# jacarvalho/mpd-public

Hardware: AMD Instinct MI355X
Metric: denoising-steps/s (higher is better)
Workload: dtype f32; 1 GPU; cfg2: EnvDense2D-RobotPointMass shape, 100 trajectories (1 context(s)) x H=64 x D=4, T=100 (+5) reverse steps, unguided, U-Net dim_mults (1, 2, 4, 8), one plan = one bench step; parallelism=single, denoising_steps_per_plan=105

## Files before the change

### include/mpdx.h

```cpp
#ifndef MPDX_H
#define MPDX_H

#include <stddef.h>
#include <stdint.h>

#ifdef __cplusplus
extern "C" {
#endif

#define MPDX_E_INVALID   (-1)
#define MPDX_E_NOTFOUND  (-2)
#define MPDX_E_STATE     (-3)

#define MPDX_MAX_LEVELS 8

typedef struct mpdx_unet mpdx_unet;

typedef struct mpdx_unet_cfg {
    int32_t state_dim;
    int32_t n_support_points;
    int32_t unet_input_dim;
    int32_t n_levels;
    int32_t dim_mults[MPDX_MAX_LEVELS];
    int32_t time_emb_dim;
// ... 148 lines not shown
    float    step;
    int32_t  max_nodes, max_iters, max_connect_steps, n_edge_checks;
    uint64_t seed;
} mpdx_rrt_opts;
int mpdx_rrt_connect(const mpdx_guide_params* gp, const mpdx_rrt_opts* opts, const float* start, const float* goal, float* nodes,
                     int32_t* parent, int32_t* count, int32_t* link, int32_t* iters, int n, void* stream);

int mpdx_rrt_paths(const mpdx_guide_params* gp, const float* start, const float* goal, const float* nodes, const int32_t* parent, const int32_t* link,
                   float* trajs_out, int32_t* path_len, int n, int max_nodes, int H, float dt, int n_edge_checks, int rounds, void* stream);

int mpdx_plan(mpdx_unet* u, const float* packed_dev, const float* timetab_dev, int T, const mpdx_step_coefs* coefs,
              int n_without_noise, float* x, const float* noise, const float* hard_start, const float* hard_goal,
              float* chain, int B, float* ws, const mpdx_guide_params* guide, int n_guide_steps, int t_start_guide,
              uint32_t* guide_flags, int n_per_ctx, uint64_t rng_seed, uint64_t rng_offset, void* stream);

int mpdx_unet_profile(mpdx_unet* u, const float* packed_dev, const float* timetab_dev, int T, const float* x, int t,
                      int B, float* ws, void* stream, int cap, float* ms_out, double* flops_out,
                      const char** names_out, int* n_out);
int mpdx_layer_trace(mpdx_unet* u, const float* packed_dev, const float* timetab_dev, const float* x, int layer, int B, float* ws,
                     void* stream, long long* stamps32);
int mpdx_fused_trace(mpdx_unet* u, const float* packed_dev, const float* timetab_dev, const float* x, int seg, int B,
                     float* ws, void* stream, long long* stamps_out, int cap, int* n_out, int* nops_out);
int mpdx_unet_time_units(mpdx_unet* u, const float* packed_dev, const float* timetab_dev, int T, const float* x, int t, int B,
                         float* ws, void* stream, int unit_first, int unit_last, int reps, float* ms_avg);
int mpdx_unet_time_without(mpdx_unet* u, const float* packed_dev, const float* timetab_dev, int T, const float* x, int t, int B,
                           float* ws, void* stream, unsigned long long skip_mask, int reps, float* ms_avg);
int mpdx_unet_unit_layer(const mpdx_unet* u, int B, int i);
int mpdx_unet_fused_program(const mpdx_unet* u, int seg);
double mpdx_unet_unit_bytes(const mpdx_unet* u, int B, int i);
int mpdx_unet_unit_is_pair(const mpdx_unet* u, int B, int i);
// ... 9 lines not shown
```

### mpd_public_amd/_lib.py

```python
from __future__ import annotations

import ctypes as C
from pathlib import Path

import os as _os

_LIB_PATH = Path(_os.environ["MPDX_LIB"]) if _os.environ.get("MPDX_LIB") else Path(__file__).resolve().parent / "libmpdx.so"
_lib = None

MAX_LEVELS = 8


class UnetCfg(C.Structure):
    _fields_ = [("state_dim", C.c_int32), ("n_support_points", C.c_int32), ("unet_input_dim", C.c_int32),
                ("n_levels", C.c_int32), ("dim_mults", C.c_int32 * MAX_LEVELS), ("time_emb_dim", C.c_int32)]


class StepCoefs(C.Structure):
    _fields_ = [("sqrt_recip_alphas_cumprod", C.c_float), ("sqrt_recipm1_alphas_cumprod", C.c_float),
                ("posterior_mean_coef1", C.c_float), ("posterior_mean_coef2", C.c_float),
                ("noise_scale", C.c_float), ("noise_std_extra", C.c_float),
                ("predict_epsilon", C.c_int32), ("clip_denoised", C.c_int32), ("ddim_k1", C.c_float), ("ddim_k2", C.c_float),
                ("guide_scale", C.c_float)]

# ... 40 lines not shown
    "mpdx_unet_num_params": (_i, [_vp]),
    "mpdx_unet_param_info": (_i, [_vp, _i, C.POINTER(C.c_char_p), C.POINTER(C.c_int32 * 3), C.POINTER(C.c_int32)]),
    "mpdx_unet_packed_floats": (_sz, [_vp]),
    "mpdx_unet_timetab_floats": (_sz, [_vp, _i]),
    "mpdx_unet_workspace_floats": (_sz, [_vp, _i]),
    "mpdx_unet_pack_param": (_i, [_vp, C.c_char_p, _vp, _sz, _vp, _vp]),
    "mpdx_unet_build_timetab": (_i, [_vp, _vp, _vp, _i, _vp, _vp]),
    "mpdx_unet_forward": (_i, [_vp, _vp, _vp, _i, _vp, _i, _vp, _i, _vp, _vp]),
    "mpdx_ddpm_step": (_i, [_vp, _vp, _vp, _i, _vp, _vp, _vp, _vp, C.POINTER(StepCoefs), _i, _i, _vp, _vp, _i, _i, _vp, _vp]),
    "mpdx_add_noise": (_i, [_vp, _vp, _vp, _vp, _f, _f, _vp, _i, _i, _i, _vp]),
    "mpdx_hard_conds": (_i, [_vp, _vp, _i, C.POINTER(C.c_int32), C.POINTER(_vp), _i, _i, _i, _vp]),
    "mpdx_q_sample": (_i, [_vp, _vp, _vp, _vp, _vp, _vp, _vp, _vp, _i, _i, _i, _i, _vp]),
    "mpdx_weighted_loss": (_i, [_vp, _vp, _vp, _vp, _vp, _i, _vp, _i, _i, _i, _vp]),
    "mpdx_plan": (_i, [_vp, _vp, _vp, _i, C.POINTER(StepCoefs), _i, _vp, _vp, _vp, _vp, _vp, _i, _vp,
                        C.POINTER(GuideParams), _i, _i, _vp, _i, C.c_uint64, C.c_uint64, _vp]),
    "mpdx_guide_step": (_i, [C.POINTER(GuideParams), _vp, _vp, _vp, _vp, _vp, _vp, _i, _i, _i, _i, _vp]),
    "mpdx_guide_step_scaled": (_i, [C.POINTER(GuideParams), _vp, _vp, _vp, _vp, _vp, _vp, _i, _i, _i, _i, _f, _vp]),
    "mpdx_guide_time": (_i, [C.POINTER(GuideParams), _vp, _vp, _vp, _i, _i, _i, _i, _i, _vp, C.POINTER(C.c_float)]),
    "mpdx_traj_metrics": (_i, [C.POINTER(GuideParams), _vp, _vp, _i, _i, _i, _i, _vp]),
    "mpdx_traj_metrics_mask": (_i, [C.POINTER(GuideParams), _vp, _vp, _vp, _i, _i, _i, _i, _vp]),
    "mpdx_guide_trace": (_i, [C.POINTER(GuideParams), _vp, _vp, _i, _i, _i, _vp, C.POINTER(C.c_longlong)]),
    "mpdx_absmax": (_i, [_vp, _vp, _i, _i, _i, _i, _vp]),
    "mpdx_sdf_grid_bake": (_i, [C.POINTER(GuideParams), _i, _vp, _vp, C.POINTER(C.c_int * 3), C.POINTER(C.c_float * 3), _f, _vp]),
    "mpdx_unet_profile": (_i, [_vp, _vp, _vp, _i, _vp, _i, _i, _vp, _vp, _i, C.POINTER(C.c_float), C.POINTER(C.c_double),
                                C.POINTER(C.c_char_p), C.POINTER(C.c_int)]),
    "mpdx_layer_trace": (_i, [_vp, _vp, _vp, _vp, _i, _i, _vp, _vp, C.POINTER(C.c_longlong)]),
    "mpdx_fused_trace": (_i, [_vp, _vp, _vp, _vp, _i, _i, _vp, _vp, C.POINTER(C.c_longlong), _i, C.POINTER(C.c_int), C.POINTER(C.c_int)]),
    "mpdx_unet_time_units": (_i, [_vp, _vp, _vp, _i, _vp, _i, _i, _vp, _vp, _i, _i, _i, C.POINTER(C.c_float)]),
    "mpdx_unet_time_without": (_i, [_vp, _vp, _vp, _i, _vp, _i, _i, _vp, _vp, C.c_uint64, _i, C.POINTER(C.c_float)]),
    "mpdx_unet_unit_layer": (_i, [_vp, _i, _i]),
# ... 66 lines not shown
```

### mpd_public_amd/csrc/fused_level.hpp

```cpp
#pragma once
#include "conv_block.hpp"
#include "fused_geom.hpp"

namespace mpdx {

#define MPDX_FUSED_SHAPES(X)                                                                                   \
    X(0, CONV_S1, 5, 1, 0, 32, 64, 1) X(1, CONV_S1, 5, 2, 1, 32, 64, 1) X(2, CONV_S1, 5, 2, 0, 32, 64, 1) X(3, CONV_DOWN, 3, 2, 0, 32, 32, 0)     \
    X(4, CONV_S1, 5, 2, 0, 64, 32, 1) X(5, CONV_S1, 5, 4, 2, 64, 32, 1) X(6, CONV_S1, 5, 4, 0, 64, 32, 1) X(7, CONV_DOWN, 3, 4, 0, 64, 16, 0)     \
    X(8, CONV_S1, 5, 16, 0, 64, 16, 1) X(9, CONV_S1, 5, 4, 16, 64, 16, 1) X(10, CONV_S1, 5, 4, 0, 64, 16, 1) X(11, CONV_UPT, 4, 4, 0, 64, 32, 0)  \
    X(12, CONV_S1, 5, 8, 0, 32, 32, 1) X(13, CONV_S1, 5, 2, 8, 32, 32, 1) X(14, CONV_S1, 5, 2, 0, 32, 32, 1) X(15, CONV_UPT, 4, 2, 0, 32, 64, 0) \
    X(16, CONV_S1, 5, 4, 0, 128, 16, 1) X(17, CONV_S1, 5, 8, 4, 128, 16, 1) X(18, CONV_S1, 5, 8, 0, 128, 16, 1) X(19, CONV_DOWN, 3, 8, 0, 128, 8, 0)
constexpr int kFusedShapeFinal = 63;

inline int fused_shape_id(int mode, int ks, int nc16, int rnc16, int cout, int L_out, int gn) {
#define X(id, M, K, N, R, CO, LO, G) if (mode == M && ks == K && nc16 == N && rnc16 == R && cout == CO && L_out == LO && gn == G) return id;
    MPDX_FUSED_SHAPES(X)
#undef X
    return -1;
}

constexpr int kFusedWaves = 4;
constexpr int kFusedThreads = 64 * kFusedWaves;

template <int MODE_, int KS_, int NC16_, int NCR_, int COUT_, int LOUT_, int GN_>
// ... 461 lines not shown
#pragma unroll
    for (int k = 0; k < kFinalPre; ++k) {
        const int idx = tid + k * kFusedThreads;
        if (k * kFusedThreads >= n) continue;
        const int ic = idx < n ? idx : 0;
        const int p = ic / a.D, d = ic - p * a.D;
        const size_t o = (size_t)b * n + ic;
        fp.xv[k] = a.x_in[o];
        if (a.fmode == 1 && !a.rng.on && a.noise) fp.nz[k] = a.noise[o];
        if (a.hs && p == 0) fp.hc[k] = a.hs[(size_t)b * a.D + d];
        if (a.hg && p == H - 1) fp.hc[k] = a.hg[(size_t)b * a.D + d];
    }
}

template <int CF = 0>
__device__ __forceinline__ void fused_final_op(const FusedArgs& a, const FusedLay& lay, const FusedOp& op, const FinalPre& fp, float* smem, int tid, int lane, int b) {
    f32x4* const sm4 = (f32x4*)smem;
    constexpr int NT_ = kFusedThreads;
    float vmax = 0.f;
    const int H = lay.H, n = H * a.D;
    const int Cf = CF ? CF : lay.Cf;
    const int wrs = Cf + 4;
    const float* const fw = smem + lay.par_off + lay.fpar_off;
    float nzr[kFinalPre];
    const bool coop = a.fmode == 1 && a.rng.on && (((a.rng.elem0 + (unsigned long long)b * (unsigned)n) & 3ull) == 0ull) && (n & 3) == 0;
    if (coop) {
        const int qidx = (tid & ~63) + (lane >> 4) * NT_ + (lane & 15) * 4;
        float z[4] = {0.f, 0.f, 0.f, 0.f};
        if (qidx < n) philox_normal4(a.rng.seed, a.rng.offset + ((a.rng.elem0 + (unsigned long long)b * (unsigned)n + (unsigned)qidx) >> 2), z);
#pragma unroll
        for (int k = 0; k < kFinalPre; ++k) {
// ... 34 lines not shown
                if (a.hs && p == 0) r = fp.hc[k];
                if (a.hg && p == H - 1) r = fp.hc[k];
            } else {
                if (a.k.clip_denoised) x0 = fminf(fmaxf(x0, -1.0f), 1.0f);
                r = __fadd_rn(__fmul_rn(a.k.posterior_mean_coef1, x0), __fmul_rn(a.k.posterior_mean_coef2, xv));
                if (a.fmode == 1) {
                    if (a.rng.on) r = __fadd_rn(r, __fmul_rn(__fmul_rn(a.k.noise_scale, coop ? nzr[k] : philox_normal_at(a.rng.seed, a.rng.offset, a.rng.elem0 + o)), a.k.noise_std_extra));
                    else if (a.noise) r = __fadd_rn(r, __fmul_rn(__fmul_rn(a.k.noise_scale, fp.nz[k]), a.k.noise_std_extra));
                    if (a.hs && p == 0) r = fp.hc[k];
                    if (a.hg && p == H - 1) r = fp.hc[k];
                }
            }
        }
        a.out[o] = r;
        if (a.chain) a.chain[o] = r;
        vmax = fmaxf(vmax, fabsf(r));
    }
    if (a.absmax) {
#pragma unroll
        for (int s = 32; s >= 1; s >>= 1) vmax = fmaxf(vmax, __shfl_xor(vmax, s, 64));
        if (lane == 0) atomicMax(a.absmax + b / a.n_per_ctx, __float_as_uint(vmax));
    }
}

template <bool SAVE>
__global__ __launch_bounds__(kFusedThreads) void fused_level_kernel(const FusedArgs a) {
#ifndef MPDX_NO_WARM_KERNARG
    warm_kernarg<(int)sizeof(FusedArgs)>();
#endif
    extern __shared__ __attribute__((aligned(16))) float smem[];
// ... 71 lines not shown
        }
        fused_conv_op<typename FusedShapeOf<SH>::type, SAVE>(a, lay, op, ring, smem, wave, lane, b, nbase, nmax, tr_base, tr);
    }
}

template <class GEOM_, int... SH>
struct FusedSeq {
    using GEOM = GEOM_;
    static constexpr int N = sizeof...(SH);
    static constexpr int ids[sizeof...(SH)] = {SH...};
    template <int I>
    static constexpr int prev_cout() {
        if constexpr (I > 0 && ids[I > 0 ? I - 1 : 0] != kFusedShapeFinal) return FusedShapeOf<ids[I > 0 ? I - 1 : 0]>::type::COUT;
        else return 0;
    }
    template <int I, bool SAVE>
    __device__ static __forceinline__ void run_from(const FusedArgs& a, const FusedLay& lay, f32x4 (&ring)[kFusedRing], FinalPre& fp, float* smem, int tid, int wave,
                                                    int lane, int b, long long* tr_base, int& tr) {
        if constexpr (I < N) {
            fused_static_op<GEOM, ids[I], I, (I + 1 < N ? ids[I + 1 < N ? I + 1 : I] : -1), prev_cout<I>(), SAVE>(a, lay, ring, fp, smem, tid, wave, lane, b, tr_base, tr);
            run_from<I + 1, SAVE>(a, lay, ring, fp, smem, tid, wave, lane, b, tr_base, tr);
        }
    }
};

template <class SEQ, bool SAVE = false>
__global__ __launch_bounds__(kFusedThreads) void fused_program_kernel(const FusedArgs a) {
#ifndef MPDX_NO_WARM_KERNARG
    warm_kernarg<(int)sizeof(FusedArgs)>();
#endif
    extern __shared__ __attribute__((aligned(16))) float smem[];
    const int tid = threadIdx.x, lane = tid & 63;
    const int wave = __builtin_amdgcn_readfirstlane(tid >> 6);
    const int b = blockIdx.x;
    int tr = 0;
    long long* const tr_base = (MPDX_TRACE_PTR(a.trace) && b == 0 && lane == 0) ? a.trace + wave * 128 : nullptr;
// ... 2 lines not shown
    f32x4 ring[kFusedRing];
    FinalPre fp;
    const FusedLay lay = fused_lay<typename SEQ::GEOM>(a);
    fused_prologue<typename SEQ::GEOM>(a, lay, smem, ring, tid, lane, wave, b, tr_base, tr);
    SEQ::template run_from<0, SAVE>(a, lay, ring, fp, smem, tid, wave, lane, b, tr_base, tr);
}

using FusedSeqDown = FusedSeq<GeomDown, 0, 1, 2, 2, 3, 4, 5, 6, 6, 7>;
using FusedSeqUpA = FusedSeq<GeomNone, 8, 9, 10, 10, 11>;
using FusedSeqUpB = FusedSeq<GeomNone, 12, 13, 14, 14, 15, 2, kFusedShapeFinal>;
using FusedSeqUpAB = FusedSeq<GeomUpAB, 8, 9, 10, 10, 11, 12, 13, 14, 14, 15, 2, kFusedShapeFinal>;
using FusedSeqDown3 = FusedSeq<GeomDown3, 0, 1, 2, 2, 3, 4, 5, 6, 6, 7, 16, 17, 18, 18, 19>;
using FusedSeqMid2 = FusedSeq<GeomNone, 16, 17, 18, 18, 19>;
using FusedSeqMid3 = FusedSeq<GeomMid3, 16, 17, 18, 18, 18, 18, 18, 18>;

}
```

### mpd_public_amd/csrc/host.hpp

```cpp
#pragma once
#include <hip/hip_runtime.h>

#include <algorithm>
#include <cmath>
#include <cstdarg>
#include <cstdio>
#include <cstdlib>
#include <cstring>
#include <mutex>
#include <set>
#include <string>
#include <unordered_map>
#include <vector>

#include "../../include/mpdx.h"
#include "conv_block.hpp"
#include "conv_ws.hpp"
#include "fused_level.hpp"
#include "switches.hpp"
#include "train_types.hpp"

namespace mpdx {

int fail(int code, const char* fmt, ...);
// ... 109 lines not shown

int pick_row_stride(int cin_pad, int mode, int L_in, int L_out, int LP);
void choose_tile(const Layer& l, int B, int& MT, int& NT);
bool layer_ksplit(const Layer& l);
int check_ready(const mpdx_unet* u);
unsigned fused_mask(int B);
bool fused_save_variant(const mpdx_unet::Fused& f);
int ensure_fused_streams(mpdx_unet* u, const float* packed, hipStream_t st);
int claim_fused_stream_jobs(mpdx_unet* u, const float* packed, const void** jobs, int* n);
int launch_final_step(const FinalArgs& fa, hipStream_t st);
int launch_conv_layer(const Layer& l, ConvArgs& a, int B, hipStream_t st);
bool pair_tile(const Layer& l1, const Layer& l2, int B, int& MT, int& NT);
int launch_conv_pair(int MT, int NT, const ConvArgs& a1, const ConvArgs& a2, const Layer& l1, const Layer& l2, hipStream_t st);
int launch_weight_stationary(int variant, const Layer& l, ConvArgs& a, const ConvArgs& a2, int B, hipStream_t st);
int launch_fused_args(const mpdx_unet::Fused& f, const FusedArgs& a, int B, hipStream_t st, bool save = false);
int launch_fused_train(const mpdx_unet::Fused& f, const FusedArgs& a, int B, hipStream_t st);
struct NoiseRng;
int launch_guide(const mpdx_guide_params* gp, float* x, float* grad_out, const float* hs, const float* hg, const uint32_t* amax_in,
                 uint32_t* amax_out, int n_per_ctx, int B, int H, int D, hipStream_t st, const float* noise = nullptr, float noise_scale = 0.f,
                 float noise_extra = 0.f, float* chain = nullptr, float guide_scale = 1.0f, const NoiseRng* rng = nullptr);

}
```

### mpd_public_amd/csrc/k_fused.hip

```cpp
#include "host.hpp"

namespace mpdx {

int launch_fused_args(const mpdx_unet::Fused& f, const FusedArgs& a, int B, hipStream_t st, bool save) {
    if (save) return launch_fused_train(f, a, B, st);
    switch (f.program) {
        case 0:
            if (int rc = raise_lds_limit((const void*)fused_program_kernel<FusedSeqDown>)) return rc;
            hipLaunchKernelGGL(fused_program_kernel<FusedSeqDown>, dim3(B), dim3(kFusedThreads), f.lds_bytes, st, a);
            break;
        case 1:
            if (int rc = raise_lds_limit((const void*)fused_program_kernel<FusedSeqUpA>)) return rc;
            hipLaunchKernelGGL(fused_program_kernel<FusedSeqUpA>, dim3(B), dim3(kFusedThreads), f.lds_bytes, st, a);
            break;
        case 2:
            if (int rc = raise_lds_limit((const void*)fused_program_kernel<FusedSeqUpB>)) return rc;
            hipLaunchKernelGGL(fused_program_kernel<FusedSeqUpB>, dim3(B), dim3(kFusedThreads), f.lds_bytes, st, a);
            break;
        case 3:
            if (int rc = raise_lds_limit((const void*)fused_program_kernel<FusedSeqUpAB>)) return rc;
            hipLaunchKernelGGL(fused_program_kernel<FusedSeqUpAB>, dim3(B), dim3(kFusedThreads), f.lds_bytes, st, a);
            break;
        case 4:
            if (int rc = raise_lds_limit((const void*)fused_program_kernel<FusedSeqMid2>)) return rc;
// ... 2 lines not shown
        case 5:
            if (int rc = raise_lds_limit((const void*)fused_program_kernel<FusedSeqDown3>)) return rc;
            hipLaunchKernelGGL(fused_program_kernel<FusedSeqDown3>, dim3(B), dim3(kFusedThreads), f.lds_bytes, st, a);
            break;
        case 6:
            if (int rc = raise_lds_limit((const void*)fused_program_kernel<FusedSeqMid3>)) return rc;
            hipLaunchKernelGGL(fused_program_kernel<FusedSeqMid3>, dim3(B), dim3(kFusedThreads), f.lds_bytes, st, a);
            break;
        default:
            if (int rc = raise_lds_limit((const void*)fused_level_kernel<false>)) return rc;
            hipLaunchKernelGGL(fused_level_kernel<false>, dim3(B), dim3(kFusedThreads), f.lds_bytes, st, a);
    }
    return 0;
}

}
```

### mpd_public_amd/csrc/mpdx.hip

```cpp
#include "host.hpp"
#include "loss.hpp"

namespace mpdx {

static thread_local char g_err[512] = "";
int fail(int code, const char* fmt, ...) {
    va_list ap;
    va_start(ap, fmt);
    vsnprintf(g_err, sizeof(g_err), fmt, ap);
    va_end(ap);
    return code;
}

int raise_lds_limit(const void* kern) {
    static std::mutex mu;
    static std::set<std::pair<int, const void*>> done;
    int dev = 0;
    HIP_TRY(hipGetDevice(&dev));
    std::lock_guard<std::mutex> lock(mu);
    if (done.count({dev, kern})) return 0;
    HIP_TRY(hipFuncSetAttribute(kern, hipFuncAttributeMaxDynamicSharedMemorySize, 160 * 1024));
    done.insert({dev, kern});
    return 0;
}
// ... 991 lines not shown
        hipLaunchKernelGGL(restream_all_kernel, dim3(64, (unsigned)u->n_jobs), dim3(256), 0, st, const_cast<float*>(packed), (const CopyJobDev*)u->jobs_dev);
    HIP_TRY(hipGetLastError());
    u->streams_for = packed; u->streams_version = u->pack_version;
    return 0;
}
int claim_fused_stream_jobs(mpdx_unet* u, const float* packed, const void** jobs, int* n) {
    *jobs = nullptr; *n = 0;
    if (u->streams_for == packed && u->streams_version == u->pack_version) return 0;
    if (int rc = ensure_stream_jobs(u)) return rc;
    *jobs = u->jobs_dev; *n = u->n_jobs;
    u->streams_for = packed; u->streams_version = u->pack_version;
    return 0;
}

bool fused_save_variant(const mpdx_unet::Fused& f) { return f.program == 0 || f.program == 3 || f.program == 5 || f.program == 6 || f.program < 0; }
static int run_fused(mpdx_unet* u, const mpdx_unet::Fused& f, const float* packed, const float* tt_row, const float* x, float* ws,
                     int B, const FinalArgs* fa, hipStream_t st) {
    const size_t slot = u->slot_floats * (size_t)B;
    auto src = [&](int s) -> const float* { return s == SRC_X ? x : (s == SRC_NONE ? nullptr : ws + slot * s); };
    if (int rc = ensure_fused_streams(u, packed, st)) return rc;
    FusedArgs a = f.tmpl;
    a.packed = packed; a.tt_row = tt_row;
    a.gsrc1 = src(f.in1); a.gsrc2 = src(f.in2);
    a.gsrc3 = f.in3 != SRC_NONE ? src(f.in3) : a.gsrc1;
    for (int k = 0; k < 3; ++k) a.gout[k] = f.gout_slot[k] >= 0 ? ws + slot * f.gout_slot[k] : nullptr;
    a.B = B;
    a.trace = (g_fused_trace && (g_fused_trace_seg < 0 || g_fused_trace_seg == (int)(&f - &u->fused[0]))) ? g_fused_trace : nullptr;
    if (f.has_final) {
        if (!fa) return fail(MPDX_E_STATE, "fused final segment needs the step arguments");
        a.x_in = fa->x_in; a.noise = fa->noise; a.hs = fa->hs; a.hg = fa->hg; a.out = fa->out; a.chain = fa->chain;
        a.absmax = fa->absmax; a.fmode = fa->mode; a.n_per_ctx = fa->n_per_ctx > 0 ? fa->n_per_ctx : B; a.k = fa->k;
        a.rng = fa->rng;
    }
    return launch_fused_args(f, a, B, st);
}


static int run_unit(mpdx_unet* u, const mpdx_unet::Unit& un, const float* packed, const float* row, const float* x, float* ws, int B,
                    const FinalArgs* fa, hipStream_t st) {
    if (un.fused >= 0) return run_fused(u, u->fused[un.fused], packed, row, x, ws, B, fa, st);
    if (un.pair) return run_pair(u, u->layers[un.layer], u->layers[un.layer + 1], packed, row, x, ws, B, st);
    return run_layer(u, u->layers[un.layer], packed, row, x, ws, B, st);
}
static double unit_flops(const mpdx_unet* u, const mpdx_unet::Unit& un, int B) {
    if (un.fused >= 0) {
        const auto& f = u->fused[un.fused];
        double fl = 0.0;
        for (int k = f.first; k < f.first + f.count; ++k) fl += layer_flops(u->layers[k], B);
// ... 248 lines not shown
static int plan_side(mpdx_unet* u, mpdx_unet::PlanSide** out) {
    mpdx_unet::PlanSide& s = u->side;
    if (!s.stream) {
        HIP_TRY(hipStreamCreateWithFlags(&s.stream, hipStreamNonBlocking));
        HIP_TRY(hipEventCreateWithFlags(&s.fork, hipEventDisableTiming));
        HIP_TRY(hipEventCreateWithFlags(&s.join, hipEventDisableTiming));
    }
    *out = &s;
    return 0;
}
static int plan_split_point(int B, int npc, int n_ctx) {
    if (sw::plan_chains() != 2 || B < 16) return 0;
    if (n_ctx >= 2) return (n_ctx / 2) * npc;
    return std::min(B - 4, ((B / 2) + 3) & ~3);
}
}

int mpdx_plan(mpdx_unet* u, const float* packed, const float* timetab, int T, const mpdx_step_coefs* coefs, int n_without_noise,
              float* x, const float* noise, const float* hard_start, const float* hard_goal, float* chain, int B, float* ws,
              const mpdx_guide_params* guide, int n_guide_steps, int t_start_guide, uint32_t* guide_flags, int n_per_ctx,
              uint64_t rng_seed, uint64_t rng_offset, void* stream) {
    if (!u || !packed || !timetab || !coefs || !x || !ws || T <= 0 || n_without_noise < 0 || B <= 0)
        return fail(MPDX_E_INVALID, "bad argument");
    if (int rc = check_ready(u)) return rc;
    hipStream_t st = (hipStream_t)stream;
    const int H = u->cfg.n_support_points, D = u->cfg.state_dim;
    const size_t n = (size_t)B * H * D;
    const int npc = n_per_ctx > 0 ? n_per_ctx : B;
    const int n_ctx = (B + npc - 1) / npc;
    const int steps = T + n_without_noise;
// ... 10 lines not shown
    const int B0 = plan_split_point(B, npc, n_ctx);
    const int nch = B0 > 0 ? 2 : 1;
    mpdx_unet::PlanSide* side = nullptr;
    if (nch == 2) {
        if (int rc = plan_side(u, &side)) return rc;
        if (int rc = ensure_fused_streams(u, packed, st)) return rc;
        HIP_TRY(hipEventRecord(side->fork, st));
        HIP_TRY(hipStreamWaitEvent(side->stream, side->fork, 0));
    }
    const int b0[2] = {0, B0}, nb[2] = {nch == 2 ? B0 : B, B - B0};
    hipStream_t sts[2] = {st, side ? side->stream : st};
    float* wss[2] = {ws, ws + u->slot_floats * (size_t)nb[0] * u->n_slots};
    struct ChainsGuard { int* p; ~ChainsGuard() { *p = 1; } } guard{&g_plan_chains};
    g_plan_chains = nch;
    bool forked = nch == 2;
    int k = 0;
    for (int i = T - 1; i >= -n_without_noise; --i, ++k) {
        const int t = i < 0 ? 0 : i;
        const bool guided = guide && i < t_start_guide;
        const float* nz = (t == 0 || !noise) ? nullptr : noise + (size_t)k * n;
        NoiseRng rng;
        memset(&rng, 0, sizeof(rng));
        if (!noise && t != 0) { rng.on = 1; rng.seed = rng_seed; rng.offset = rng_offset; rng.elem0 = (unsigned long long)(k + 1) * n; }
        float* ch = chain ? chain + (size_t)(k + 1) * n : nullptr;
        uint32_t* fl = guided ? guide_flags + (size_t)k * (n_guide_steps + 1) * n_ctx : nullptr;
        if (nch == 2 && !forked) {
            HIP_TRY(hipEventRecord(side->fork, st));
            HIP_TRY(hipStreamWaitEvent(side->stream, side->fork, 0));
            forked = true;
        }
// ... 1 lines not shown
            const size_t eo = (size_t)b0[c] * H * D;
            FinalArgs fa;
            memset(&fa, 0, sizeof(fa));
            fa.x_in = x + eo; fa.out = x + eo;
            fa.k = coefs[t];
            fa.n_per_ctx = npc;
            if (!guided) {
                fa.rng = rng;
                fa.rng.elem0 += eo;
                fa.noise = nz ? nz + eo : nullptr;
                fa.hs = hard_start ? hard_start + (size_t)b0[c] * D : nullptr; fa.hg = hard_goal ? hard_goal + (size_t)b0[c] * D : nullptr;
                fa.chain = ch ? ch + eo : nullptr; fa.mode = 1;
            } else {
                fa.mode = 2; fa.absmax = fl + b0[c] / npc;
            }
            if (int rc = run_unet_and_final(u, packed, timetab, T, x + eo, t, nb[c], wss[c], fa, sts[c])) return rc;
        }
        if (guided) {
            if (nch == 2) {
                HIP_TRY(hipEventRecord(side->join, side->stream));
                HIP_TRY(hipStreamWaitEvent(st, side->join, 0));
                forked = false;
            }
            for (int j = 0; j < n_guide_steps; ++j) {
                const bool last = j == n_guide_steps - 1;
                if (int rc = launch_guide(guide, x, nullptr, hard_start, hard_goal, fl + (size_t)j * n_ctx, fl + (size_t)(j + 1) * n_ctx, npc, B, H,
                                          D, st, last ? nz : nullptr, coefs[t].noise_scale, coefs[t].noise_std_extra, last ? ch : nullptr,
                                          coefs[t].guide_scale, last ? &rng : nullptr))
                    return rc;
            }
// ... 2 lines not shown
            if (dbg >= 2) {
                hipError_t e = hipStreamSynchronize(st);
                if (e == hipSuccess && nch == 2) e = hipStreamSynchronize(side->stream);
                if (e != hipSuccess) return fail((int)e, "mpdx_plan: loop iteration %d (t=%d%s) faulted: %s", k, t, guided ? ", guided" : "", hipGetErrorString(e));
            }
            hipError_t e = hipGetLastError();
            if (e != hipSuccess) return fail((int)e, "mpdx_plan: launch in loop iteration %d (t=%d%s) failed: %s", k, t, guided ? ", guided" : "", hipGetErrorString(e));
        }
    }
    if (nch == 2 && forked) {
        HIP_TRY(hipEventRecord(side->join, side->stream));
        HIP_TRY(hipStreamWaitEvent(st, side->join, 0));
    }
    HIP_TRY(hipGetLastError());
    return 0;
}

int mpdx_unet_profile(mpdx_unet* u, const float* packed, const float* timetab, int T, const float* x, int t, int B, float* ws,
                      void* stream, int cap, float* ms_out, double* flops_out, const char** names_out, int* n_out) {
    if (!u || !packed || !timetab || !x || !ws || !ms_out || !n_out) return fail(MPDX_E_INVALID, "null argument");
    if (int rc = check_ready(u)) return rc;
    if (t < 0 || t >= T) return fail(MPDX_E_INVALID, "timestep %d outside [0,%d)", t, T);
    hipStream_t st = (hipStream_t)stream;
    bool fin_fused = false;
    const auto units = current_units(u, B, &fin_fused);
    const bool need_final = !fin_fused;
    const int nl = (int)units.size() + (need_final ? 1 : 0);
    if (cap < nl) return fail(MPDX_E_INVALID, "need room for %d launches", nl);
    static float* scratch = nullptr;
    static size_t scratch_n = 0;
// ... 275 lines not shown
```

### mpd_public_amd/diffusion_model.py

```python
from __future__ import annotations

from copy import copy

import torch
import torch.nn as nn

from . import _lib
from .sample_functions import apply_hard_conditioning, ddpm_sample_fn, extract, step_coefs
from .schedules import diffusion_buffers


def make_timesteps(batch_size, i, device):
    t = torch.full((batch_size,), i, device=device, dtype=torch.long)
    t._mpdx_value = int(i)
    t._mpdx_version = t._version
    return t


def timestep_hint(t):
    v = getattr(t, "_mpdx_value", None)
    return v if v is not None and getattr(t, "_mpdx_version", -1) == t._version else None


class GaussianDiffusionModel(nn.Module):
# ... 115 lines not shown
        npc = int(n_per_context or B)
        gp_ref, flags, n_gs, t_sg = None, None, 0, 0
        if int(n_guide_steps) <= 0:
            guide = None
        if guide is not None:
            import ctypes as C
            gp_ref = C.byref(guide.device_params(dev))
            n_gs = int(n_guide_steps)
            t_sg = int(min(t_start_guide, T + 1)) if t_start_guide != float("inf") else T + 1
            flags = torch.empty(steps * (n_gs + 1) * ((B + npc - 1) // npc), dtype=torch.int32, device=dev)
        _lib.check(_lib.load().mpdx_plan(hdl, packed.data_ptr(), tab.data_ptr(), T, coefs, n0,
                                         x.data_ptr(), noise_ptr, _lib.ptr(hs), _lib.ptr(hg), _lib.ptr(chain), B,
                                         ws.data_ptr(), gp_ref, n_gs, t_sg, _lib.ptr(flags), npc, rng_seed, rng_offset,
                                         _lib.current_stream()), "mpdx_plan")
        return x, chain

    def predict_noise_from_start(self, x_t, t, x0):
        if self.predict_epsilon:
            return x0
        return (extract(self.sqrt_recip_alphas_cumprod, t, x_t.shape) * x_t - x0) / extract(self.sqrt_recipm1_alphas_cumprod, t, x_t.shape)

    def predict_start_from_noise(self, x_t, t, noise):
        if not self.predict_epsilon:
            return noise
        return extract(self.sqrt_recip_alphas_cumprod, t, x_t.shape) * x_t - extract(self.sqrt_recipm1_alphas_cumprod, t, x_t.shape) * noise

    def q_posterior(self, x_start, x_t, t):
        mean = extract(self.posterior_mean_coef1, t, x_t.shape) * x_start + extract(self.posterior_mean_coef2, t, x_t.shape) * x_t
        return mean, extract(self.posterior_variance, t, x_t.shape), extract(self.posterior_log_variance_clipped, t, x_t.shape)

# ... 230 lines not shown
```

Measured before the change: 5733 denoising-steps/s.

## Merge up-path fused program with next step's down-path into one launch

Adds a fused_step_kernel that runs the final up-path fused program (including the DDPM update) and then, in the same block, the next timestep's down-path fused program. The updated sample goes straight into LDS as the next network input. This saves one kernel launch per denoising step and the global round trip of the sample between steps. A slot-redirection planner moves intermediate buffers when the down half would overwrite tensors the up half still reads. The merge only applies for a single chain, unguided runs and B no larger than the CU count. It raises LDS use per block and adds complex slot-aliasing logic.

```diff
diff --git a/include/mpdx.h b/include/mpdx.h
--- a/include/mpdx.h
+++ b/include/mpdx.h
@@ -186,6 +186,8 @@
               float* chain, int B, float* ws, const mpdx_guide_params* guide, int n_guide_steps, int t_start_guide,
               uint32_t* guide_flags, int n_per_ctx, uint64_t rng_seed, uint64_t rng_offset, void* stream);
 
+int mpdx_plan_merged_steps(mpdx_unet* u, int B, int T, int n_without_noise, int guided, int t_start_guide);
+
 int mpdx_unet_profile(mpdx_unet* u, const float* packed_dev, const float* timetab_dev, int T, const float* x, int t,
                       int B, float* ws, void* stream, int cap, float* ms_out, double* flops_out,
                       const char** names_out, int* n_out);
diff --git a/mpd_public_amd/_lib.py b/mpd_public_amd/_lib.py
--- a/mpd_public_amd/_lib.py
+++ b/mpd_public_amd/_lib.py
@@ -78,6 +78,7 @@
     "mpdx_weighted_loss": (_i, [_vp, _vp, _vp, _vp, _vp, _i, _vp, _i, _i, _i, _vp]),
     "mpdx_plan": (_i, [_vp, _vp, _vp, _i, C.POINTER(StepCoefs), _i, _vp, _vp, _vp, _vp, _vp, _i, _vp,
                         C.POINTER(GuideParams), _i, _i, _vp, _i, C.c_uint64, C.c_uint64, _vp]),
+    "mpdx_plan_merged_steps": (_i, [_vp, _i, _i, _i, _i, _i]),
     "mpdx_guide_step": (_i, [C.POINTER(GuideParams), _vp, _vp, _vp, _vp, _vp, _vp, _i, _i, _i, _i, _vp]),
     "mpdx_guide_step_scaled": (_i, [C.POINTER(GuideParams), _vp, _vp, _vp, _vp, _vp, _vp, _i, _i, _i, _i, _f, _vp]),
     "mpdx_guide_time": (_i, [C.POINTER(GuideParams), _vp, _vp, _vp, _i, _i, _i, _i, _i, _vp, C.POINTER(C.c_float)]),
diff --git a/mpd_public_amd/csrc/fused_level.hpp b/mpd_public_amd/csrc/fused_level.hpp
--- a/mpd_public_amd/csrc/fused_level.hpp
+++ b/mpd_public_amd/csrc/fused_level.hpp
@@ -499,7 +499,8 @@
 }
 
 template <int CF = 0>
-__device__ __forceinline__ void fused_final_op(const FusedArgs& a, const FusedLay& lay, const FusedOp& op, const FinalPre& fp, float* smem, int tid, int lane, int b) {
+__device__ __forceinline__ void fused_final_op(const FusedArgs& a, const FusedLay& lay, const FusedOp& op, const FinalPre& fp, float* smem, int tid, int lane, int b,
+                                               float* hand = nullptr, int hand_rs = 0) {
     f32x4* const sm4 = (f32x4*)smem;
     constexpr int NT_ = kFusedThreads;
     float vmax = 0.f;
@@ -564,6 +565,7 @@
         }
         a.out[o] = r;
         if (a.chain) a.chain[o] = r;
+        if (hand) hand[(p + 2) * hand_rs + d] = r;
         vmax = fmaxf(vmax, fabsf(r));
     }
     if (a.absmax) {
@@ -665,12 +667,12 @@
         if constexpr (I > 0 && ids[I > 0 ? I - 1 : 0] != kFusedShapeFinal) return FusedShapeOf<ids[I > 0 ? I - 1 : 0]>::type::COUT;
         else return 0;
     }
-    template <int I, bool SAVE>
+    template <int I, bool SAVE, int END = N>
     __device__ static __forceinline__ void run_from(const FusedArgs& a, const FusedLay& lay, f32x4 (&ring)[kFusedRing], FinalPre& fp, float* smem, int tid, int wave,
                                                     int lane, int b, long long* tr_base, int& tr) {
-        if constexpr (I < N) {
+        if constexpr (I < END) {
             fused_static_op<GEOM, ids[I], I, (I + 1 < N ? ids[I + 1 < N ? I + 1 : I] : -1), prev_cout<I>(), SAVE>(a, lay, ring, fp, smem, tid, wave, lane, b, tr_base, tr);
-            run_from<I + 1, SAVE>(a, lay, ring, fp, smem, tid, wave, lane, b, tr_base, tr);
+            run_from<I + 1, SAVE, END>(a, lay, ring, fp, smem, tid, wave, lane, b, tr_base, tr);
         }
     }
 };
@@ -703,4 +705,110 @@
 using FusedSeqMid2 = FusedSeq<GeomNone, 16, 17, 18, 18, 19>;
 using FusedSeqMid3 = FusedSeq<GeomMid3, 16, 17, 18, 18, 18, 18, 18, 18>;
 
-}
+constexpr int kStepUpBase = GeomDown3::g.par_off + GeomDown3::g.par_floats;
+constexpr int kStepUpFloats = 16000;
+
+struct FusedStepArgs {
+    const float* packed;
+    const float* tt_up;
+    const float* tt_dn;
+    const float* gsrc1; const float* gsrc2; const float* gsrc3;
+    float* gout[3];
+    const float* x_in; const float* noise; const float* hs; const float* hg;
+    float* out; float* chain;
+    int up_sbase[kMaxFusedOps], dn_sbase[kMaxFusedOps];
+    int up_gpar_off, up_par_floats, up_tt_lo, up_in_clear;
+    int dn_gpar_off, dn_tt_lo;
+    int D, B;
+    mpdx_step_coefs k;
+    NoiseRng rng;
+};
+
+static_assert(sizeof(FusedStepArgs) == 360, "DESIGN.md section 3 states this size");
+template <class UP, class DN>
+__global__ __launch_bounds__(kFusedThreads) __attribute__((amdgpu_waves_per_eu(3))) void fused_step_kernel(const FusedStepArgs m) {
+#ifndef MPDX_NO_WARM_KERNARG
+    warm_kernarg<(int)sizeof(FusedStepArgs)>();
+#endif
+    extern __shared__ __attribute__((aligned(16))) float smem[];
+    using UG = typename UP::GEOM;
+    using DG = typename DN::GEOM;
+    static_assert(UG::has && DG::has && UP::ids[UP::N - 1] == kFusedShapeFinal && UP::N >= 3, "two static programs, the first ends in the final op");
+    constexpr FusedGeom gu = UG::g, gd = DG::g;
+    static_assert(gd.par_floats >= 0 && gd.gc1 < 0 && gd.c3 == 0, "the down half stages nothing but the network input");
+    static_assert((kStepUpBase & 3) == 0 && gd.par_off + gd.par_floats <= kStepUpBase && gd.tt_off + gd.tt_n <= gd.par_off, "the down half ends where the up half begins");
+    static_assert(gu.par_off + gu.fpar_off + (16 * (gu.Cf + 4) + 16 + 3) / 4 * 4 <= kStepUpFloats, "the up half's LDS size");
+    const int tid = threadIdx.x, lane = tid & 63;
+    const int wave = __builtin_amdgcn_readfirstlane(tid >> 6);
+    const int b = blockIdx.x;
+    int tr = 0;
+    float* const smd = smem;
+    int ubase = kStepUpBase;
+    asm volatile("" : "+s"(ubase));
+    float* const smu = smem + ubase;
+    f32x4* const smd4 = (f32x4*)smd;
+    FusedArgs au = {};
+    au.packed = m.packed;
+    au.tt_row = m.tt_up;
+    au.gsrc1 = m.gsrc1; au.gsrc2 = m.gsrc2; au.gsrc3 = m.gsrc3;
+    au.gc1 = gu.gc1; au.gc2 = gu.gc2; au.in_clear = m.up_in_clear;
+    au.gpar_off = m.up_gpar_off; au.par_floats = m.up_par_floats; au.tt_lo = m.up_tt_lo;
+    au.B = m.B; au.nops = UP::N;
+#pragma unroll
+    for (int i = 0; i < UP::N - 1; ++i) au.ops[i].sbase = m.up_sbase[i];
+    {
+        using U0 = typename FusedShapeOf<UP::ids[0]>::type;
+        au.msmask[0] = U0::MSn - 1; au.slen[0] = U0::SLEN;
+    }
+    au.x_in = m.x_in; au.noise = m.noise; au.hs = m.hs; au.hg = m.hg; au.out = m.out; au.chain = m.chain;
+    au.D = m.D; au.fmode = 1; au.n_per_ctx = m.B; au.k = m.k; au.rng = m.rng;
+    f32x4 ring[kFusedRing];
+    FinalPre fp;
+    const FusedLay layu = fused_lay<UG>(au);
+    {
+        const f32x4 z = {0.f, 0.f, 0.f, 0.f};
+        for (int i = tid; i < gd.in_rows * gd.in_rs4; i += kFusedThreads) smd4[gd.in_off4 + i] = z;
+    }
+    fused_prologue<UG>(au, layu, smu, ring, tid, lane, wave, b, nullptr, tr);
+    constexpr int kPar4 = (gd.par_floats + gd.tt_n) / 4, PK = (kPar4 + kFusedThreads - 1) / kFusedThreads;
+    constexpr int npar4 = gd.par_floats / 4, ntt4 = gd.tt_n / 4;
+    f32x4 pv[PK];
+#pragma unroll
+    for (int k = 0; k < PK; ++k) {
+        const int idx = tid + k * kFusedThreads;
+        if (k * kFusedThreads >= kPar4) continue;
+        const float* src = idx < npar4 ? m.packed + m.dn_gpar_off + (size_t)idx * 4 : m.tt_dn + m.dn_tt_lo + (size_t)(idx - npar4 < ntt4 ? idx - npar4 : 0) * 4;
+        pv[k] = *(const f32x4*)src;
+    }
+    __builtin_amdgcn_sched_barrier(0);
+    UP::template run_from<0, false, 1>(au, layu, ring, fp, smu, tid, wave, lane, b, nullptr, tr);
+#pragma unroll
+    for (int k = 0; k < PK; ++k) {
+        const int idx = tid + k * kFusedThreads;
+        if (idx < npar4) smd4[(gd.par_off >> 2) + idx] = pv[k];
+        else if (idx - npar4 < ntt4) smd4[(gd.tt_off >> 2) + idx - npar4] = pv[k];
+    }
+    UP::template run_from<1, false, UP::N - 2>(au, layu, ring, fp, smu, tid, wave, lane, b, nullptr, tr);
+    {
+        constexpr int I = UP::N - 2;
+        fused_final_prefetch(au, layu, fp, tid, b);
+        const FusedOp op = fused_static_desc<UG, I, false>(au);
+        using N0 = typename FusedShapeOf<DN::ids[0]>::type;
+        const int nbase = (m.dn_sbase[0] + (wave & (N0::MSn < kFusedWaves ? N0::MSn - 1 : kFusedWaves - 1)) * (N0::SLEN * 256)) * 4;
+        fused_conv_op<typename FusedShapeOf<UP::ids[I]>::type, false>(au, layu, op, ring, smu, wave, lane, b, nbase, N0::SLEN - 1, nullptr, tr);
+    }
+    {
+        const FusedOp op = fused_static_desc<UG, UP::N - 1, false>(au);
+        fused_final_op<UP::template prev_cout<UP::N - 1>()>(au, layu, op, fp, smu, tid, lane, b, smd + gd.in_off4 * 4, gd.in_rs4 * 4);
+    }
+    lds_barrier();
+    FusedArgs ad = {};
+    ad.packed = m.packed; ad.tt_row = m.tt_dn; ad.B = m.B; ad.nops = DN::N; ad.gc1 = m.D;
+    ad.gout[0] = m.gout[0]; ad.gout[1] = m.gout[1]; ad.gout[2] = m.gout[2];
+#pragma unroll
+    for (int i = 0; i < DN::N; ++i) ad.ops[i].sbase = m.dn_sbase[i];
+    const FusedLay layd = fused_lay<DG>(ad);
+    DN::template run_from<0, false>(ad, layd, ring, fp, smd, tid, wave, lane, b, nullptr, tr);
+}
+
+}
diff --git a/mpd_public_amd/csrc/host.hpp b/mpd_public_amd/csrc/host.hpp
--- a/mpd_public_amd/csrc/host.hpp
+++ b/mpd_public_amd/csrc/host.hpp
@@ -147,6 +147,8 @@
 int launch_conv_pair(int MT, int NT, const ConvArgs& a1, const ConvArgs& a2, const Layer& l1, const Layer& l2, hipStream_t st);
 int launch_weight_stationary(int variant, const Layer& l, ConvArgs& a, const ConvArgs& a2, int B, hipStream_t st);
 int launch_fused_args(const mpdx_unet::Fused& f, const FusedArgs& a, int B, hipStream_t st, bool save = false);
+int launch_fused_step(const mpdx_unet::Fused& up, const mpdx_unet::Fused& dn, const FusedArgs& au, const FusedArgs& ad, int B, hipStream_t st);
+size_t fused_step_lds_bytes();
 int launch_fused_train(const mpdx_unet::Fused& f, const FusedArgs& a, int B, hipStream_t st);
 struct NoiseRng;
 int launch_guide(const mpdx_guide_params* gp, float* x, float* grad_out, const float* hs, const float* hg, const uint32_t* amax_in,
diff --git a/mpd_public_amd/csrc/k_fused.hip b/mpd_public_amd/csrc/k_fused.hip
--- a/mpd_public_amd/csrc/k_fused.hip
+++ b/mpd_public_amd/csrc/k_fused.hip
@@ -40,4 +40,26 @@
     return 0;
 }
 
+size_t fused_step_lds_bytes() { return (size_t)(kStepUpBase + kStepUpFloats) * sizeof(float); }
+int launch_fused_step(const mpdx_unet::Fused& up, const mpdx_unet::Fused& dn, const FusedArgs& au, const FusedArgs& ad, int B, hipStream_t st) {
+    if (up.program != 3 || dn.program != 5 || au.fmode != 1 || au.absmax || up.lds_bytes > (size_t)kStepUpFloats * sizeof(float) ||
+        dn.lds_bytes > (size_t)kStepUpBase * sizeof(float) || fused_step_lds_bytes() > 160 * 1024)
+        return fail(MPDX_E_STATE, "step-merged launch: programs %d + %d, final mode %d do not qualify", up.program, dn.program, au.fmode);
+    FusedStepArgs m;
+    memset(&m, 0, sizeof(m));
+    m.packed = au.packed; m.tt_up = au.tt_row; m.tt_dn = ad.tt_row;
+    m.gsrc1 = au.gsrc1; m.gsrc2 = au.gsrc2; m.gsrc3 = au.gsrc3;
+    for (int k = 0; k < 3; ++k) m.gout[k] = ad.gout[k];
+    m.x_in = au.x_in; m.noise = au.noise; m.hs = au.hs; m.hg = au.hg; m.out = au.out; m.chain = au.chain;
+    for (int k = 0; k < au.nops; ++k) m.up_sbase[k] = au.ops[k].sbase;
+    for (int k = 0; k < ad.nops; ++k) m.dn_sbase[k] = ad.ops[k].sbase;
+    m.up_gpar_off = au.gpar_off; m.up_par_floats = au.par_floats; m.up_tt_lo = au.tt_lo; m.up_in_clear = au.in_clear;
+    m.dn_gpar_off = ad.gpar_off; m.dn_tt_lo = ad.tt_lo;
+    m.D = au.D; m.B = B; m.k = au.k; m.rng = au.rng;
+    const void* kern = (const void*)fused_step_kernel<FusedSeqUpAB, FusedSeqDown3>;
+    if (int rc = raise_lds_limit(kern)) return rc;
+    hipLaunchKernelGGL((fused_step_kernel<FusedSeqUpAB, FusedSeqDown3>), dim3(B), dim3(kFusedThreads), fused_step_lds_bytes(), st, m);
+    return 0;
 }
+
+}
diff --git a/mpd_public_amd/csrc/mpdx.hip b/mpd_public_amd/csrc/mpdx.hip
--- a/mpd_public_amd/csrc/mpdx.hip
+++ b/mpd_public_amd/csrc/mpdx.hip
@@ -1029,12 +1029,11 @@
 }
 
 bool fused_save_variant(const mpdx_unet::Fused& f) { return f.program == 0 || f.program == 3 || f.program == 5 || f.program == 6 || f.program < 0; }
-static int run_fused(mpdx_unet* u, const mpdx_unet::Fused& f, const float* packed, const float* tt_row, const float* x, float* ws,
-                     int B, const FinalArgs* fa, hipStream_t st) {
+static int fill_fused_args(mpdx_unet* u, const mpdx_unet::Fused& f, const float* packed, const float* tt_row, const float* x, float* ws, int B, const FinalArgs* fa,
+                           FusedArgs& a) {
     const size_t slot = u->slot_floats * (size_t)B;
     auto src = [&](int s) -> const float* { return s == SRC_X ? x : (s == SRC_NONE ? nullptr : ws + slot * s); };
-    if (int rc = ensure_fused_streams(u, packed, st)) return rc;
-    FusedArgs a = f.tmpl;
+    a = f.tmpl;
     a.packed = packed; a.tt_row = tt_row;
     a.gsrc1 = src(f.in1); a.gsrc2 = src(f.in2);
     a.gsrc3 = f.in3 != SRC_NONE ? src(f.in3) : a.gsrc1;
@@ -1047,6 +1046,13 @@
         a.absmax = fa->absmax; a.fmode = fa->mode; a.n_per_ctx = fa->n_per_ctx > 0 ? fa->n_per_ctx : B; a.k = fa->k;
         a.rng = fa->rng;
     }
+    return 0;
+}
+static int run_fused(mpdx_unet* u, const mpdx_unet::Fused& f, const float* packed, const float* tt_row, const float* x, float* ws,
+                     int B, const FinalArgs* fa, hipStream_t st) {
+    if (int rc = ensure_fused_streams(u, packed, st)) return rc;
+    FusedArgs a;
+    if (int rc = fill_fused_args(u, f, packed, tt_row, x, ws, B, fa, a)) return rc;
     return launch_fused_args(f, a, B, st);
 }
 
@@ -1325,6 +1331,151 @@
     if (n_ctx >= 2) return (n_ctx / 2) * npc;
     return std::min(B - 4, ((B / 2) + 3) & ~3);
 }
+
+struct StepMerge {
+    bool ok = false;
+    int seg_dn = -1, seg_up = -1;
+    int slot_old = -1, slot_alt = -1, gout_k = -1;
+    std::vector<int> readers;
+};
+static int device_cu_count() {
+    int dev = 0, n = 0;
+    if (hipGetDevice(&dev) != hipSuccess || hipDeviceGetAttribute(&n, hipDeviceAttributeMultiprocessorCount, dev) != hipSuccess) {
+        (void)hipGetLastError();
+        return 0;
+    }
+    return n;
+}
+static StepMerge plan_step_merge(const mpdx_unet* u, int B, const std::vector<mpdx_unet::Unit>& units, bool one_chain) {
+    StepMerge m;
+    const int dbg = debug_fuse_level();
+    auto off = [&](const char* why) {
+        if (dbg) fprintf(stderr, "[mpdx] step merge B=%d: off (%s)\n", B, why);
+        return StepMerge();
+    };
+#ifdef MPDX_NO_STEP_MERGE
+    return off("compiled out");
+#endif
+    if (u->masked()) return off("padded horizon");
+    if (units.size() < 3 || units.front().fused < 0 || units.back().fused < 0) return off("the pass does not start and end with a fused program");
+    m.seg_dn = units.front().fused; m.seg_up = units.back().fused;
+    const mpdx_unet::Fused& dn = u->fused[m.seg_dn];
+    const mpdx_unet::Fused& up = u->fused[m.seg_up];
+    if (dn.program != 5 || up.program != 3 || !up.has_final || dn.has_final || dn.first != 0) return off("not the static programs 5 + 3");
+    for (size_t i = 1; i + 1 < units.size(); ++i)
+        if (units[i].fused >= 0) return off("a fused program between the two");
+    if (!one_chain) return off("two chains");
+    if (B > device_cu_count()) return off("more trajectories than CUs");
+    if (up.lds_bytes > (size_t)kStepUpFloats * sizeof(float) || dn.lds_bytes > (size_t)kStepUpBase * sizeof(float) || fused_step_lds_bytes() > 160 * 1024)
+        return off("LDS regions");
+    struct Buf { int slot, L, C, k; };
+    std::vector<Buf> up_r, dn_w;
+    const Layer& u0 = u->layers[up.first];
+    if (up.in1 >= 0) up_r.push_back({up.in1, u0.L_in, u0.c1, 0});
+    if (up.in2 >= 0) up_r.push_back({up.in2, u0.L_in, u0.c2, 1});
+    if (up.in3 >= 0 && up.in3_consumer >= 0) up_r.push_back({up.in3, u->layers[up.in3_consumer].L_in, u->layers[up.in3_consumer].c2, 2});
+    for (int k = 0; k < dn.tmpl.nops; ++k) {
+        const FusedOp& o = dn.tmpl.ops[k];
+        if (o.shape == kFusedShapeFinal || o.gdst < 0) continue;
+        const Layer& l = u->layers[dn.op_layer[k]];
+        dn_w.push_back({dn.gout_slot[o.gdst], l.L_out, l.cout, o.gdst});
+    }
+    auto clash = [&](const Buf& w) {
+        for (const Buf& r : up_r)
+            if (r.slot == w.slot && (r.L != w.L || r.C != w.C)) return true;
+        return false;
+    };
+    const int last_dn = dn.first + dn.count - 1, first_up = up.first;
+    auto reads = [&](const Layer& l, int s) { return l.src1 == s || l.src2 == s || l.res == s; };
+    for (Buf& w : dn_w) {
+        if (!clash(w)) continue;
+        if (m.slot_alt >= 0 || w.slot != u->layers[last_dn].dst || w.L != u->layers[last_dn].L_out) return off("a clashing buffer that cannot move");
+        m.slot_old = w.slot; m.gout_k = w.k;
+        bool closed = false;
+        for (int i = last_dn + 1; i < first_up && !closed; ++i) {
+            if (reads(u->layers[i], m.slot_old)) m.readers.push_back(i);
+            closed = u->layers[i].dst == m.slot_old;
+        }
+        if (!closed || m.readers.empty()) return off("the moved tensor's readers are not bounded by a writer");
+        const int r_last = m.readers.back();
+        for (int s = 0; s < u->n_slots && m.slot_alt < 0; ++s) {
+            if (s == m.slot_old || s == u->xpad_slot) continue;
+            bool free_ = up.in1 != s && up.in2 != s && up.in3 != s && dn.in1 != s && dn.in2 != s && dn.in3 != s;
+            for (int k = 0; k < 3; ++k) free_ = free_ && up.gout_slot[k] != s && dn.gout_slot[k] != s;
+            for (int i = last_dn + 1; i <= r_last && free_; ++i) free_ = !reads(u->layers[i], s) && u->layers[i].dst != s;
+            for (int i = r_last + 1; i < first_up && free_; ++i) {
+                if (reads(u->layers[i], s)) free_ = false;
+                if (u->layers[i].dst == s) break;
+            }
+            if (free_) m.slot_alt = s;
+        }
+        if (m.slot_alt < 0) return off("no free slot for the moved tensor");
+        w.slot = m.slot_alt;
+        if (clash(w)) return off("the moved tensor clashes again");
+    }
+    if (dbg) {
+        for (const Buf& r : up_r) fprintf(stderr, "[mpdx] step merge B=%d: up reads slot %d as %dx%d\n", B, r.slot, r.L, r.C);
+        for (const Buf& w : dn_w) fprintf(stderr, "[mpdx] step merge B=%d: down writes slot %d as %dx%d\n", B, w.slot, w.L, w.C);
+        if (m.slot_alt >= 0) {
+            fprintf(stderr, "[mpdx] step merge B=%d: moved slot %d -> %d, readers:", B, m.slot_old, m.slot_alt);
+            for (int i : m.readers) fprintf(stderr, " %s", u->layers[i].name.c_str());
+            fprintf(stderr, "\n");
+        }
+        fprintf(stderr, "[mpdx] step merge B=%d: on\n", B);
+    }
+    m.ok = true;
+    return m;
+}
+
+static int run_pass_merged(mpdx_unet* u, const std::vector<mpdx_unet::Unit>& units, const StepMerge& sm, const float* packed, const float* timetab, const float* x,
+                           int t, int t_next, int B, float* ws, FinalArgs& fa, hipStream_t st, bool down_done) {
+    const float* row = timetab + (size_t)t * u->tt_row;
+    const size_t slot = u->slot_floats * (size_t)B;
+    const bool moved = down_done && sm.slot_alt >= 0;
+    auto is_reader = [&](int li) { return std::find(sm.readers.begin(), sm.readers.end(), li) != sm.readers.end(); };
+    auto redirect = [&](int li) {
+        Layer l = u->layers[li];
+        if (is_reader(li)) {
+            if (l.src1 == sm.slot_old) l.src1 = sm.slot_alt;
+            if (l.src2 == sm.slot_old) l.src2 = sm.slot_alt;
+            if (l.res == sm.slot_old) l.res = sm.slot_alt;
+        }
+        return l;
+    };
+    for (size_t i = 0; i < units.size(); ++i) {
+        const mpdx_unet::Unit& un = units[i];
+        if (i == 0) {
+            if (!down_done)
+                if (int rc = run_unit(u, un, packed, row, x, ws, B, &fa, st)) return rc;
+            continue;
+        }
+        if (i + 1 < units.size()) {
+            if (!moved || !(is_reader(un.layer) || (un.pair && is_reader(un.layer + 1)))) {
+                if (int rc = run_unit(u, un, packed, row, x, ws, B, &fa, st)) return rc;
+            } else if (un.pair) {
+                const Layer l1 = redirect(un.layer), l2 = redirect(un.layer + 1);
+                if (int rc = run_pair(u, l1, l2, packed, row, x, ws, B, st)) return rc;
+            } else {
+                const Layer l1 = redirect(un.layer);
+                if (int rc = run_layer(u, l1, packed, row, x, ws, B, st)) return rc;
+            }
+            continue;
+        }
+        if (t_next < 0) {
+            if (int rc = run_unit(u, un, packed, row, x, ws, B, &fa, st)) return rc;
+            continue;
+        }
+        const mpdx_unet::Fused& dn = u->fused[sm.seg_dn];
+        const mpdx_unet::Fused& up = u->fused[sm.seg_up];
+        if (int rc = ensure_fused_streams(u, packed, st)) return rc;
+        FusedArgs au, ad;
+        if (int rc = fill_fused_args(u, up, packed, row, x, ws, B, &fa, au)) return rc;
+        if (int rc = fill_fused_args(u, dn, packed, timetab + (size_t)t_next * u->tt_row, x, ws, B, nullptr, ad)) return rc;
+        if (sm.slot_alt >= 0) ad.gout[sm.gout_k] = ws + slot * sm.slot_alt;
+        if (int rc = launch_fused_step(up, dn, au, ad, B, st)) return rc;
+    }
+    return 0;
+}
 }
 
 int mpdx_plan(mpdx_unet* u, const float* packed, const float* timetab, int T, const mpdx_step_coefs* coefs, int n_without_noise,
@@ -1365,6 +1516,13 @@
     struct ChainsGuard { int* p; ~ChainsGuard() { *p = 1; } } guard{&g_plan_chains};
     g_plan_chains = nch;
     bool forked = nch == 2;
+    std::vector<mpdx_unet::Unit> units;
+    StepMerge sm;
+    if (nch == 1 && steps > 1) {
+        units = current_units(u, B, nullptr);
+        sm = plan_step_merge(u, B, units, true);
+    }
+    bool down_done = false;
     int k = 0;
     for (int i = T - 1; i >= -n_without_noise; --i, ++k) {
         const int t = i < 0 ? 0 : i;
@@ -1396,6 +1554,14 @@
             } else {
                 fa.mode = 2; fa.absmax = fl + b0[c] / npc;
             }
+            if (sm.ok) {
+                const bool merge_next = !guided && k + 1 < steps && fa.mode == 1 && !fa.absmax;
+                const int t_next = merge_next ? (i - 1 < 0 ? 0 : i - 1) : -1;
+                if (t < 0 || t >= T) return fail(MPDX_E_INVALID, "timestep %d outside [0,%d)", t, T);
+                if (int rc = run_pass_merged(u, units, sm, packed, timetab, x, t, t_next, B, ws, fa, st, down_done)) return rc;
+                down_done = merge_next;
+                continue;
+            }
             if (int rc = run_unet_and_final(u, packed, timetab, T, x + eo, t, nb[c], wss[c], fa, sts[c])) return rc;
         }
         if (guided) {
@@ -1428,6 +1594,17 @@
     }
     HIP_TRY(hipGetLastError());
     return 0;
+}
+
+int mpdx_plan_merged_steps(mpdx_unet* u, int B, int T, int n_without_noise, int guided, int t_start_guide) {
+    if (!u || B <= 0 || T <= 0 || n_without_noise < 0) return 0;
+    const int steps = T + n_without_noise;
+    if (steps < 2) return 0;
+    if (!plan_step_merge(u, B, current_units(u, B, nullptr), plan_split_point(B, B, 1) == 0).ok) return 0;
+    int n = 0, k = 0;
+    for (int i = T - 1; i >= -n_without_noise; --i, ++k)
+        if (!(guided && i < t_start_guide) && k + 1 < steps) ++n;
+    return n;
 }
 
 int mpdx_unet_profile(mpdx_unet* u, const float* packed, const float* timetab, int T, const float* x, int t, int B, float* ws,
diff --git a/mpd_public_amd/diffusion_model.py b/mpd_public_amd/diffusion_model.py
--- a/mpd_public_amd/diffusion_model.py
+++ b/mpd_public_amd/diffusion_model.py
@@ -153,6 +153,16 @@
                                          ws.data_ptr(), gp_ref, n_gs, t_sg, _lib.ptr(flags), npc, rng_seed, rng_offset,
                                          _lib.current_stream()), "mpdx_plan")
         return x, chain
+
+    def plan_merged_steps(self, n_samples, n_diffusion_steps_without_noise=0, guide=None, n_guide_steps=1,
+                          t_start_guide=float("inf"), fused=True):
+        if not fused:
+            return 0
+        T, B = self.n_diffusion_steps, int(n_samples)
+        hdl = self.model._handle()
+        guided = guide is not None and int(n_guide_steps) > 0
+        t_sg = int(min(t_start_guide, T + 1)) if t_start_guide != float("inf") else T + 1
+        return int(_lib.load().mpdx_plan_merged_steps(hdl, B, T, int(n_diffusion_steps_without_noise), int(guided), t_sg))
 
     def predict_noise_from_start(self, x_t, t, x0):
         if self.predict_epsilon:
```

After: 5834 denoising-steps/s, median of 6. 1.02x the previous value.
